# Circuitscape/Circuitscape.jl

Measured on AMD Instinct MI355X. Metric: pair-solves/sec (AMG-PCG, setup amortised over 100 pairs) on 10000x10000 raster pairwise, higher is better.
Workload: dtype f64

## Files before the change

circuitscape.jl_amd/csrc/lattice.h:

```cpp
#pragma once
#include "stencil.h"

namespace csgpu {

__device__ __forceinline__ int lat_tile(int i, int nc) {
  const int t = i / 3;
  return t < nc ? t : nc - 1;
}

template <class T>
__global__ __launch_bounds__(256) void lattice_q_fill_kernel(int64_t n, int R, int Rc, int Cc, const int* __restrict__ agg,
                                                             const int* __restrict__ qrp, const int* __restrict__ qci,
                                                             const T* __restrict__ qva, T* __restrict__ q,
                                                             int* __restrict__ bad) {
  for (int64_t node = (int64_t)blockIdx.x * 256 + threadIdx.x; node < n; node += (int64_t)gridDim.x * 256) {
    const int i = (int)(node % R), j = (int)(node / R);
    const int I = lat_tile(i, Rc), J = lat_tile(j, Cc);
    {
      const int a = agg[node];
      const int dI = a % Rc - I, dJ = a / Rc - J;
      if (dI < -1 || dI > 1 || dJ < -1 || dJ > 1) {
        atomicOr(bad, 1);
        continue;
      }
    }
    T row[9];
#pragma unroll
    for (int s = 0; s < 9; ++s) row[s] = T(0);
    for (int k = qrp[node]; k < qrp[node + 1]; ++k) {
      const int c = qci[k];
      const int dI = c % Rc - I, dJ = c / Rc - J;
      if (dI < -1 || dI > 1 || dJ < -1 || dJ > 1) {
        atomicOr(bad, 2);
        continue;
      }
      const int slot = (dJ + 1) * 3 + (dI + 1);
#pragma unroll
      for (int s = 0; s < 9; ++s)
        if (s == slot) row[s] = qva[k];
    }
#pragma unroll
    for (int s = 0; s < 9; ++s) q[node * 9 + s] = row[s];
  }
}

template <class T>
inline bool lattice_q_from_csr(const Csr<T>& Q, const int* agg, int R, int C, LatticeQ<T>& out, hipStream_t st) {
  const int64_t n = (int64_t)R * C;
  const int Rc = (R + 1) / 3, Cc = (C + 1) / 3;
  if (Q.nrows != n || Rc < 2 || Cc < 2 || (int64_t)Rc * Cc != Q.ncols) return false;
  DBuf q((size_t)n * 9 * sizeof(T));
  DBuf bad = dalloc<int>(1);
  CS_HIP(hipMemsetAsync(bad.p, 0, sizeof(int), st));
  hipLaunchKernelGGL((lattice_q_fill_kernel<T>), dim3(grid_for(n)), dim3(256), 0, st, n, R, Rc, Cc, agg, Q.rp(), Q.ci(),
                     Q.va(), dptr<T>(q), dptr<int>(bad));
  check_launch("index-free Q");
  if (read_int(dptr<int>(bad), st) != 0) return false;
  out.n = n;
  out.R = R;
  out.C = C;
  out.Rc = Rc;
  out.Cc = Cc;
  out.q = std::move(q);
  return true;
}

template <class T>
struct RestrictArgs {
  int R, C, Rc, Cc;
  int nstrips, nseg, segc;
  const T* q;
  const T* b;
  T* bc;
  const int* skip;
};

template <class T, int K, int NT>
struct RestrictShape {
  static constexpr int VEC = 16 / (int)sizeof(T);
  static constexpr int CPL = K < VEC ? K : VEC;
  static constexpr int LPR = K / CPL;
  static constexpr int TIC = NT / LPR;
  static constexpr int FR = 3 * TIC + 8;
  static constexpr int BU = (FR * LPR + NT - 1) / NT;
  static constexpr int QU = (FR * 9 + NT - 1) / NT;
};

template <class T, int K, int NT>
__global__ __launch_bounds__(NT) void lattice_restrict_kernel(RestrictArgs<T> a) {
  typedef RestrictShape<T, K, NT> SH;
  constexpr int CPL = SH::CPL, LPR = SH::LPR, TIC = SH::TIC, FR = SH::FR, BU = SH::BU, QU = SH::QU;
  typedef SpmvVec<T, CPL> XV;
  __shared__ XV s_b[3][FR * LPR];
  __shared__ T s_q[3][FR * 9];
  if (a.skip && *a.skip) return;
  const int tid = threadIdx.x;
  const int t = tid / LPR, lq = tid % LPR, c0 = lq * CPL;
  const int ntiles = a.nstrips * a.nseg;
  int t_first = blockIdx.x, t_last = ntiles, t_step = gridDim.x;
  if ((gridDim.x & 7) == 0) {
    const int xcd = blockIdx.x & 7, chunk = (ntiles + 7) >> 3;
    t_first = xcd * chunk + (blockIdx.x >> 3);
    t_last = min(ntiles, (xcd + 1) * chunk);
    t_step = gridDim.x >> 3;
  }
  for (int tile = t_first; tile < t_last; tile += t_step) {
    const int si = tile % a.nstrips, sj = tile / a.nstrips;
    const int Ic0 = si * TIC;
    const int Jc0 = sj * a.segc, Jc1 = min(a.Cc, Jc0 + a.segc);
    const int Ic = Ic0 + t;
    const bool row_on = Ic < a.Rc;
    const int f0 = max(3 * (Ic0 - 1), 0);
    const int last_tile = min(Ic0 + TIC, a.Rc - 1);
    const int f1 = last_tile >= a.Rc - 1 ? a.R : 3 * last_tile + 3;
    const int nfr = f1 - f0;
    const int fc0 = max(3 * (Jc0 - 1), 0);
    const int fc1 = Jc1 >= a.Cc - 1 ? a.C : 3 * Jc1 + 3;
    int rlo[3], rhi[3];
#pragma unroll
    for (int d = 0; d < 3; ++d) {
      const int tI = Ic - 1 + d;
      const bool on = row_on && tI >= 0 && tI < a.Rc;
      rlo[d] = on ? 3 * tI - f0 : 0;
      rhi[d] = on ? (tI >= a.Rc - 1 ? a.R : 3 * tI + 3) - f0 : 0;
    }
    XV breg[BU];
    T qreg[QU];
    auto load_column = [&](int f) {
      const int64_t base = (int64_t)f * a.R + f0;
#pragma unroll
      for (int u = 0; u < BU; ++u) {
        const int e = tid + u * NT;
        XV v;
#pragma unroll
        for (int q = 0; q < CPL; ++q) v.e[q] = T(0);
        if (e < nfr * LPR) v = *reinterpret_cast<const XV*>(a.b + (size_t)(base + e / LPR) * K + (e % LPR) * CPL);
        breg[u] = v;
      }
#pragma unroll
      for (int u = 0; u < QU; ++u) {
        const int e = tid + u * NT;
        qreg[u] = e < nfr * 9 ? a.q[base * 9 + e] : T(0);
      }
    };
    auto store_column = [&](int f) {
      const int slot = f % 3;
#pragma unroll
      for (int u = 0; u < BU; ++u) {
        const int e = tid + u * NT;
        if (e < FR * LPR) s_b[slot][e] = breg[u];
      }
#pragma unroll
      for (int u = 0; u < QU; ++u) {
        const int e = tid + u * NT;
        if (e < FR * 9) s_q[slot][e] = qreg[u];
      }
    };
    T acc[3][CPL];
#pragma unroll
    for (int d = 0; d < 3; ++d)
#pragma unroll
      for (int q = 0; q < CPL; ++q) acc[d][q] = T(0);
    auto emit = [&](int Jc, const T* v) {
      if (row_on && Jc >= Jc0 && Jc < Jc1) {
        XV o;
#pragma unroll
        for (int q = 0; q < CPL; ++q) o.e[q] = v[q];
        *reinterpret_cast<XV*>(a.bc + ((size_t)Jc * a.Rc + Ic) * K + c0) = o;
      }
    };
    __syncthreads();
    load_column(fc0);
    int Jf = lat_tile(fc0, a.Cc);
    for (int f = fc0; f < fc1; ++f) {
      store_column(f);
      if (f + 1 < fc1) load_column(f + 1);
      __syncthreads();
      const int Jn = lat_tile(f, a.Cc);
      if (Jn != Jf) {
        emit(Jf - 1, acc[0]);
#pragma unroll
        for (int q = 0; q < CPL; ++q) {
          acc[0][q] = acc[1][q];
          acc[1][q] = acc[2][q];
          acc[2][q] = T(0);
        }
        Jf = Jn;
      }
      const XV* sb = s_b[f % 3];
      const T* sq = s_q[f % 3];
#pragma unroll
      for (int d = 0; d < 3; ++d) {
        const int sI = (1 - d) + 1;
        for (int r = rlo[d]; r < rhi[d]; ++r) {
          const XV bv = sb[r * LPR + lq];
          const T* qr = sq + r * 9;
          const T wm = qr[0 * 3 + sI];
          const T w0 = qr[1 * 3 + sI];
          const T wp = qr[2 * 3 + sI];
#pragma unroll
          for (int q = 0; q < CPL; ++q) {
            acc[0][q] = fma(wm, bv.e[q], acc[0][q]);
            acc[1][q] = fma(w0, bv.e[q], acc[1][q]);
            acc[2][q] = fma(wp, bv.e[q], acc[2][q]);
          }
        }
      }
    }
    emit(Jf - 1, acc[0]);
    emit(Jf, acc[1]);
    emit(Jf + 1, acc[2]);
  }
}

inline int lattice_segc() {
  const int v = knobs().restrict_seg;
  return v < 2 ? 2 : v;
}

template <class T>
struct RupdRestrictOpts {
  const int* restart = nullptr;
  const int* src = nullptr;
  const int* dst = nullptr;
  const int* isrc = nullptr;
  const int* idst = nullptr;
  int icols = 0;
  T* xsol = nullptr;
};

template <class T>
struct RupdRestrictArgs : RupdRestrictOpts<T> {
  int64_t n;
  int R, C, Rc, Cc;
  int nstrips, nseg, segc;
  const T* rows;
  const T* q;
  const T* p;
  const T* r_in = nullptr;
  T* r_out;
  T* bc;
  const CgScalars* S = nullptr;
  double* partials = nullptr;
  const int* skip = nullptr;
};

template <class T, int K, int NT>
struct RupdRestrictShape {
  typedef RestrictShape<T, K, NT> RS;
  static constexpr int CPL = RS::CPL, LPR = RS::LPR, TIC = RS::TIC, FR = RS::FR;
  static constexpr int PR = FR + 2;
  static constexpr int RG = NT / LPR;
  static constexpr int BU = (FR + RG - 1) / RG;
  static constexpr int PU = (PR * LPR + NT - 1) / NT;
  static constexpr int MU = (PR * 5 + NT - 1) / NT;
  static constexpr int QU = (FR * 9 + NT - 1) / NT;
  static constexpr size_t lds_bytes = (size_t)3 * PR * LPR * 16 + (size_t)3 * PR * 5 * sizeof(T) + (size_t)FR * LPR * 16 +
                                      (size_t)FR * 9 * sizeof(T) + (size_t)(NT / 64) * K * sizeof(double);
};

template <class T, int K, int NT, bool APPLY = false, bool XUP = false>
__global__ __launch_bounds__(NT) void lattice_rupd_restrict_kernel(RupdRestrictArgs<T> a) {
  static_assert(!(APPLY && XUP), "the solution update belongs to the residual update");
  typedef RupdRestrictShape<T, K, NT> SH;
  constexpr int CPL = SH::CPL, LPR = SH::LPR, TIC = SH::TIC, FR = SH::FR, PR = SH::PR, BU = SH::BU, PU = SH::PU, MU = SH::MU,
                QU = SH::QU;
  typedef SpmvVec<T, CPL> XV;
  __shared__ XV s_p[3][PR * LPR];
  __shared__ T s_m[3][PR * 5];
  __shared__ XV s_b[FR * LPR];
  __shared__ T s_q[FR * 9];
  __shared__ double s_red[APPLY ? 1 : (NT / 64) * K];
  if (a.S && a.S->all_done) return;
  if (a.skip && *a.skip) return;
  const int tid = threadIdx.x;
  const int t = tid / LPR, lq = tid % LPR, c0 = lq * CPL;
  const int row0 = t * BU;
  T alpha[CPL];
#pragma unroll
  for (int qq = 0; qq < CPL; ++qq) alpha[qq] = APPLY ? T(0) : (T)a.S->alpha[c0 + qq];
  double dot_acc[CPL];
  bool fresh[CPL];
  int64_t nsrc[CPL], ndst[CPL];
#pragma unroll
  for (int qq = 0; qq < CPL; ++qq) {
    dot_acc[qq] = 0.0;
    fresh[qq] = !APPLY && !XUP && a.restart && a.restart[c0 + qq] != 0;
    nsrc[qq] = fresh[qq] ? a.src[c0 + qq] : -1;
    ndst[qq] = fresh[qq] ? a.dst[c0 + qq] : -1;
    if (nsrc[qq] == ndst[qq]) nsrc[qq] = ndst[qq] = -1;
  }
  const bool synth_in = !APPLY && !XUP && a.isrc != nullptr;
  int64_t is_[CPL], id_[CPL];
#pragma unroll
  for (int qq = 0; qq < CPL; ++qq) {
    const bool on = synth_in && c0 + qq < a.icols && a.isrc[c0 + qq] != a.idst[c0 + qq];
    is_[qq] = on ? a.isrc[c0 + qq] : -1;
    id_[qq] = on ? a.idst[c0 + qq] : -1;
  }
  const int ntiles = a.nstrips * a.nseg;
  int t_first = blockIdx.x, t_last = ntiles, t_step = gridDim.x;
  if ((gridDim.x & 7) == 0) {
    const int xcd = blockIdx.x & 7, chunk = (ntiles + 7) >> 3;
    t_first = xcd * chunk + (blockIdx.x >> 3);
    t_last = min(ntiles, (xcd + 1) * chunk);
    t_step = gridDim.x >> 3;
  }
  for (int tile = t_first; tile < t_last; tile += t_step) {
    const int si = tile % a.nstrips, sj = tile / a.nstrips;
    const int Ic0 = si * TIC;
    const int Jc0 = sj * a.segc, Jc1 = min(a.Cc, Jc0 + a.segc);
    const int Ic = Ic0 + t;
    const bool row_on = Ic < a.Rc;
    const int f0 = max(3 * (Ic0 - 1), 0);
    const int last_tile = min(Ic0 + TIC, a.Rc - 1);
    const int f1 = last_tile >= a.Rc - 1 ? a.R : 3 * last_tile + 3;
    const int nfr = f1 - f0;
    const int fc0 = max(3 * (Jc0 - 1), 0);
    const int fc1 = Jc1 >= a.Cc - 1 ? a.C : 3 * Jc1 + 3;
    const int o0 = 3 * Ic0, o1 = (Ic0 + TIC >= a.Rc) ? a.R : 3 * (Ic0 + TIC);
    const int oc0 = 3 * Jc0, oc1 = (Jc1 >= a.Cc) ? a.C : 3 * Jc1;
    int rlo[3], rhi[3];
#pragma unroll
    for (int d = 0; d < 3; ++d) {
      const int tI = Ic - 1 + d;
      const bool on = row_on && tI >= 0 && tI < a.Rc;
      rlo[d] = on ? 3 * tI - f0 : 0;
      rhi[d] = on ? (tI >= a.Rc - 1 ? a.R : 3 * tI + 3) - f0 : 0;
    }
    XV preg[PU];
    T mreg[MU];
    XV rreg[BU];
    XV xreg[XUP ? BU : 1];
    T qreg[QU];
    auto load_pm = [&](int f) {
      const int64_t base = (int64_t)f * a.R + f0 - 1;
#pragma unroll
      for (int u = 0; u < PU; ++u) {
        const int e = tid + u * NT;
        XV v;
#pragma unroll
        for (int qq = 0; qq < CPL; ++qq) v.e[qq] = T(0);
        const int64_t id = base + e / LPR;
        if (e < (nfr + 2) * LPR && id >= 0 && id < a.n) v = *reinterpret_cast<const XV*>(a.p + (size_t)id * K + (e % LPR) * CPL);
        preg[u] = v;
      }
#pragma unroll
      for (int u = 0; u < MU; ++u) {
        const int e = tid + u * NT;
        const int64_t g = base * 5 + e;
        mreg[u] = (e < (nfr + 2) * 5 && g >= 0 && g < a.n * 5) ? a.rows[g] : T(0);
      }
    };
    auto store_pm = [&](int slot) {
#pragma unroll
      for (int u = 0; u < PU; ++u) {
        const int e = tid + u * NT;
        if (e < PR * LPR) s_p[slot][e] = preg[u];
      }
#pragma unroll
      for (int u = 0; u < MU; ++u) {
        const int e = tid + u * NT;
        if (e < PR * 5) s_m[slot][e] = mreg[u];
      }
    };
    auto load_rq = [&](int f) {
      const int64_t base = (int64_t)f * a.R + f0;
#pragma unroll
      for (int u = 0; u < BU; ++u) {
        const int row = row0 + u;
        XV v;
#pragma unroll
        for (int qq = 0; qq < CPL; ++qq) v.e[qq] = T(0);
        if (!APPLY && f < fc1 && row < nfr) {
          const int64_t id = base + row;
          if (synth_in) {
#pragma unroll
            for (int qq = 0; qq < CPL; ++qq) v.e[qq] = id == is_[qq] ? T(-1) : (id == id_[qq] ? T(1) : T(0));
          } else {
            v = *reinterpret_cast<const XV*>(a.r_in + (size_t)id * K + c0);
          }
        }
        rreg[u] = v;
        if constexpr (XUP) {
          XV xv;
#pragma unroll
          for (int qq = 0; qq < CPL; ++qq) xv.e[qq] = T(0);
          const int fr = f0 + row;
          if (f >= oc0 && f < oc1 && row < nfr && fr >= o0 && fr < o1)
            xv = *reinterpret_cast<const XV*>(a.xsol + (size_t)(base + row) * K + c0);
          xreg[u] = xv;
        }
      }
#pragma unroll
      for (int u = 0; u < QU; ++u) {
        const int e = tid + u * NT;
        qreg[u] = (f < fc1 && e < nfr * 9) ? a.q[base * 9 + e] : T(0);
      }
    };
    T acc[3][CPL];
#pragma unroll
    for (int d = 0; d < 3; ++d)
#pragma unroll
      for (int qq = 0; qq < CPL; ++qq) acc[d][qq] = T(0);
    auto emit = [&](int Jc, const T* v) {
      if (row_on && Jc >= Jc0 && Jc < Jc1) {
        XV o;
#pragma unroll
        for (int qq = 0; qq < CPL; ++qq) o.e[qq] = v[qq];
        *reinterpret_cast<XV*>(a.bc + ((size_t)Jc * a.Rc + Ic) * K + c0) = o;
      }
    };
    __syncthreads();
    load_pm(fc0 - 1);
    store_pm(0);
    load_pm(fc0);
    store_pm(1);
    load_pm(fc0 + 1);
    load_rq(fc0);
    int Jf = lat_tile(fc0, a.Cc);
    int sm = 0, sc = 1, sp = 2;
    for (int f = fc0; f < fc1; ++f) {
      store_pm(sp);
      load_pm(f + 2);
      XV rv[BU];
      XV xv[XUP ? BU : 1];
      T qv[QU];
#pragma unroll
      for (int u = 0; u < BU; ++u) rv[u] = rreg[u];
      if constexpr (XUP) {
#pragma unroll
        for (int u = 0; u < BU; ++u) xv[u] = xreg[u];
      }
#pragma unroll
      for (int u = 0; u < QU; ++u) qv[u] = qreg[u];
      load_rq(f + 1);
      __syncthreads();
      const T* mp = s_m[sm];
      const T* mc = s_m[sc];
      const XV* xm = s_p[sm];
      const XV* x0 = s_p[sc];
      const XV* xp = s_p[sp];
      const bool col_owned = f >= oc0 && f < oc1;
      T sacc[BU][CPL];
      XV ctr[BU];
#pragma unroll
      for (int dj = 0; dj < 3; ++dj) {
        const XV* xcol = dj == 0 ? xm : (dj == 1 ? x0 : xp);
        XV win[BU + 2];
#pragma unroll
        for (int k = 0; k < BU + 2; ++k) {
#pragma unroll
          for (int qq = 0; qq < CPL; ++qq) win[k].e[qq] = T(0);
          if (row0 + k < nfr + 2) win[k] = xcol[(row0 + k) * LPR + lq];
        }
#pragma unroll
        for (int u = 0; u < BU; ++u) {
          const int row = row0 + u;
          if (row < nfr) {
            const int me = 5 * (row + 1);
            T w0, w1, w2;
            if (dj == 0) {
              w0 = mp[me - 5 + 4];
              w1 = mp[me + 3];
              w2 = mp[me + 5 + 2];
            } else if (dj == 1) {
              w0 = mc[me - 5 + 1];
              w1 = mc[me + 0];
              w2 = mc[me + 1];
            } else {
              w0 = mc[me + 2];
              w1 = mc[me + 3];
              w2 = mc[me + 4];
            }
#pragma unroll
            for (int qq = 0; qq < CPL; ++qq) {
              T sv = dj == 0 ? w0 * win[u].e[qq] : fma(w0, win[u].e[qq], sacc[u][qq]);
              sv = fma(w1, win[u + 1].e[qq], sv);
              sacc[u][qq] = fma(w2, win[u + 2].e[qq], sv);
            }
            if (dj == 1) ctr[u] = win[u + 1];
          }
        }
      }
#pragma unroll
      for (int u = 0; u < BU; ++u) {
        const int row = row0 + u;
        if (row < nfr) {
          XV rn;
#pragma unroll
          for (int qq = 0; qq < CPL; ++qq)
            rn.e[qq] = APPLY ? sacc[u][qq] : (fresh[qq] ? T(0) : rv[u].e[qq] - alpha[qq] * sacc[u][qq]);
          const int fr = f0 + row;
          const bool owned = col_owned && fr >= o0 && fr < o1;
          if (owned) {
#pragma unroll
            for (int qq = 0; qq < CPL; ++qq) dot_acc[qq] += (double)rn.e[qq] * (double)rn.e[qq];
          }
          const int64_t id = (int64_t)f * a.R + fr;
#pragma unroll
          for (int qq = 0; qq < CPL; ++qq)
            if (fresh[qq]) rn.e[qq] = id == nsrc[qq] ? T(-1) : (id == ndst[qq] ? T(1) : T(0));
          s_b[row * LPR + lq] = APPLY ? ctr[u] : rn;
          if (owned) dia_store(reinterpret_cast<XV*>(a.r_out + (size_t)id * K + c0), rn);
          if constexpr (XUP) {
            if (owned) {
              XV xn;
              const XV pc = x0[(row + 1) * LPR + lq];
#pragma unroll
              for (int qq = 0; qq < CPL; ++qq) xn.e[qq] = fma(alpha[qq], pc.e[qq], xv[u].e[qq]);
              dia_store(reinterpret_cast<XV*>(a.xsol + (size_t)id * K + c0), xn);
            }
          }
        }
      }
#pragma unroll
      for (int u = 0; u < QU; ++u) {
        const int e = tid + u * NT;
        if (e < FR * 9) s_q[e] = qv[u];
      }
      __syncthreads();
      const int Jn = lat_tile(f, a.Cc);
      if (Jn != Jf) {
        emit(Jf - 1, acc[0]);
#pragma unroll
        for (int qq = 0; qq < CPL; ++qq) {
          acc[0][qq] = acc[1][qq];
          acc[1][qq] = acc[2][qq];
          acc[2][qq] = T(0);
        }
        Jf = Jn;
      }
#pragma unroll
      for (int d = 0; d < 3; ++d) {
        const int sI = (1 - d) + 1;
        for (int r = rlo[d]; r < rhi[d]; ++r) {
          const XV bv = s_b[r * LPR + lq];
          const T* qr = s_q + r * 9;
          const T wm = qr[0 * 3 + sI];
          const T w0 = qr[1 * 3 + sI];
          const T wp = qr[2 * 3 + sI];
#pragma unroll
          for (int qq = 0; qq < CPL; ++qq) {
            acc[0][qq] = fma(wm, bv.e[qq], acc[0][qq]);
            acc[1][qq] = fma(w0, bv.e[qq], acc[1][qq]);
            acc[2][qq] = fma(wp, bv.e[qq], acc[2][qq]);
          }
        }
      }
      const int s0 = sm;
      sm = sc;
      sc = sp;
      sp = s0;
    }
    emit(Jf - 1, acc[0]);
    emit(Jf, acc[1]);
    emit(Jf + 1, acc[2]);
  }
  if (APPLY || !a.partials) return;
  if constexpr (!APPLY) {
    const int lane = tid & 63, w = tid >> 6;
    __syncthreads();
#pragma unroll
    for (int qq = 0; qq < CPL; ++qq) {
      double v = dot_acc[qq];
#pragma unroll
      for (int o = 32; o >= LPR; o >>= 1) v += __shfl_xor(v, o, 64);
      if (lane < LPR) s_red[w * K + lane * CPL + qq] = v;
    }
    __syncthreads();
    if (tid < K) {
      double ssum = 0.0;
#pragma unroll
      for (int ww = 0; ww < NT / 64; ++ww) ssum += s_red[ww * K + tid];
      a.partials[(size_t)blockIdx.x * K + tid] = ssum;
    }
  }
}

#ifndef CSGPU_FUSED_NT
#define CSGPU_FUSED_NT 512
#endif
constexpr int kFusedNT = CSGPU_FUSED_NT;
template <class T, int K>
constexpr bool lattice_rupd_restrict_fits() {
  return K >= 16 && RupdRestrictShape<T, K, kFusedNT>::lds_bytes <= (kFusedNT >= 512 ? 160 : 80) * 1024;
}

template <class T, int K>
inline int lattice_rupd_restrict_grid(const LatticeQ<T>& Q, int& nstrips, int& nseg, int& segc) {
  constexpr int NT = kFusedNT;
  segc = std::min(std::max(knobs().fused_seg, 2), Q.Cc);
  nstrips = ceil_div(Q.Rc, RestrictShape<T, K, NT>::TIC);
  while (segc > 16 && (int64_t)nstrips * ceil_div(Q.Cc, segc) < 1024) segc /= 2;
  nseg = ceil_div(Q.Cc, segc);
  int64_t g = (int64_t)nstrips * nseg;
  if (g > 16384) g = 16384;
  if (g >= 64) g &= ~(int64_t)7;
  return (int)std::max<int64_t>(g, 1);
}

template <class T, int K>
inline int lattice_rupd_args(const Dia<T>& D, const LatticeQ<T>& Q, const T* p, T* r_out, T* bc, RupdRestrictArgs<T>& a) {
  a.n = D.n;
  a.R = Q.R;
  a.C = Q.C;
  a.Rc = Q.Rc;
  a.Cc = Q.Cc;
  a.rows = D.data();
  a.q = Q.data();
  a.p = p;
  a.r_out = r_out;
  a.bc = bc;
  return lattice_rupd_restrict_grid<T, K>(Q, a.nstrips, a.nseg, a.segc);
}

template <class T, int K>
inline int lattice_rupd_restrict(const Dia<T>& D, const LatticeQ<T>& Q, const CgScalars* S, const T* p, const T* r_in, T* r_out,
                                 T* bc, double* partials, hipStream_t st, const RupdRestrictOpts<T>& o = RupdRestrictOpts<T>()) {
  CS_REQUIRE(!o.xsol || (!o.restart && !o.src && !o.dst && !o.isrc && !o.idst), CSGPU_INTERNAL,
             "fused residual update: the solution update takes a stored residual");
  if constexpr (!lattice_rupd_restrict_fits<T, K>()) {
    return 0;
  } else {
    RupdRestrictArgs<T> a;
    const int g = lattice_rupd_args<T, K>(D, Q, p, r_out, bc, a);
    a.r_in = r_in;
    a.S = S;
    a.partials = partials;
    static_cast<RupdRestrictOpts<T>&>(a) = o;
    if (o.xsol)
      hipLaunchKernelGGL((lattice_rupd_restrict_kernel<T, K, kFusedNT, false, true>), dim3(g), dim3(kFusedNT), 0, st, a);
    else
      hipLaunchKernelGGL((lattice_rupd_restrict_kernel<T, K, kFusedNT>), dim3(g), dim3(kFusedNT), 0, st, a);
    return partials ? g : 0;
  }
}

template <class T, int K>
inline bool lattice_apply_restrict(const Dia<T>& D, const LatticeQ<T>& Q, const T* x, T* y, T* bc, const int* skip,
                                   hipStream_t st) {
  if constexpr (!lattice_rupd_restrict_fits<T, K>()) {
    return false;
  } else {
    RupdRestrictArgs<T> a;
    const int g = lattice_rupd_args<T, K>(D, Q, x, y, bc, a);
    a.skip = skip;
    hipLaunchKernelGGL((lattice_rupd_restrict_kernel<T, K, kFusedNT, true>), dim3(g), dim3(kFusedNT), 0, st, a);
    return true;
  }
}

template <class T, int K>
__global__ __launch_bounds__(64) void lattice_restrict_pairs_kernel(int R, int Rc, int Cc, const T* __restrict__ q,
                                                                    const int* __restrict__ src, const int* __restrict__ dst,
                                                                    int ncols, T* __restrict__ bc) {
  const int c = threadIdx.x;
  if (c >= ncols || c >= K || src[c] == dst[c]) return;
#pragma unroll 1
  for (int which = 0; which < 2; ++which) {
    const int64_t node = which == 0 ? src[c] : dst[c];
    const T sign = which == 0 ? T(-1) : T(1);
    const int i = (int)(node % R), j = (int)(node / R);
    const int I = lat_tile(i, Rc), J = lat_tile(j, Cc);
    for (int dj = 0; dj < 3; ++dj)
      for (int di = 0; di < 3; ++di) {
        const int Ic = I + di - 1, Jc = J + dj - 1;
        if (Ic < 0 || Ic >= Rc || Jc < 0 || Jc >= Cc) continue;
        const T w = q[(size_t)node * 9 + dj * 3 + di];
        T* at = bc + ((size_t)Jc * Rc + Ic) * K + c;
        *at = fma(w, sign, *at);
      }
  }
}

template <class T, int K>
inline void lattice_restrict_pairs(const LatticeQ<T>& Q, const int* src, const int* dst, int ncols, T* bc, hipStream_t st) {
  CS_HIP(hipMemsetAsync(bc, 0, (size_t)Q.Rc * Q.Cc * K * sizeof(T), st));
  hipLaunchKernelGGL((lattice_restrict_pairs_kernel<T, K>), dim3(1), dim3(64), 0, st, Q.R, Q.Rc, Q.Cc, Q.data(), src, dst, ncols,
                     bc);
}

template <class T, int K>
inline void lattice_restrict(const LatticeQ<T>& Q, const T* b, T* bc, const int* skip, hipStream_t st) {
  constexpr int NT = 128;
  RestrictArgs<T> a;
  a.R = Q.R;
  a.C = Q.C;
  a.Rc = Q.Rc;
  a.Cc = Q.Cc;
  a.segc = std::min(lattice_segc(), Q.Cc);
  a.nstrips = ceil_div(Q.Rc, RestrictShape<T, K, NT>::TIC);
  a.nseg = ceil_div(Q.Cc, a.segc);
  a.q = Q.data();
  a.b = b;
  a.bc = bc;
  a.skip = skip;
  int64_t g = (int64_t)a.nstrips * a.nseg;
  if (g > 65536) g = 65536;
  if (g >= 64) g &= ~(int64_t)7;
  hipLaunchKernelGGL((lattice_restrict_kernel<T, K, NT>), dim3((int)std::max<int64_t>(g, 1)), dim3(NT), 0, st, a);
}

}
```

circuitscape.jl_amd/csrc/stencil.h:

```cpp
#pragma once
#include "blas1.h"
#include "spmv.h"

namespace csgpu {

#ifndef CSGPU_DIA_NT
#define CSGPU_DIA_NT 0
#endif
template <class T, int N>
__device__ __forceinline__ void dia_store(SpmvVec<T, N>* p, const SpmvVec<T, N>& v) {
#if CSGPU_DIA_NT >= 1 && defined(__HIPCC__)
  typedef T VT __attribute__((ext_vector_type(N)));
  VT t;
#pragma unroll
  for (int q = 0; q < N; ++q) t[q] = v.e[q];
  __builtin_nontemporal_store(t, reinterpret_cast<VT*>(p));
#else
  *p = v;
#endif
}
template <class T, int N>
__device__ __forceinline__ SpmvVec<T, N> dia_load(const SpmvVec<T, N>* p) {
#if CSGPU_DIA_NT >= 2 && defined(__HIPCC__)
  typedef T VT __attribute__((ext_vector_type(N)));
  const VT t = __builtin_nontemporal_load(reinterpret_cast<const VT*>(p));
  SpmvVec<T, N> v;
#pragma unroll
  for (int q = 0; q < N; ++q) v.e[q] = t[q];
  return v;
#else
  return *p;
#endif
}


__device__ __forceinline__ int dia_slot(int64_t d, int R) {
  if (d == 0) return 0;
  if (d == 1) return 1;
  if (d == R - 1) return 2;
  if (d == R) return 3;
  if (d == R + 1) return 4;
  return -1;
}

template <class T>
__global__ __launch_bounds__(256) void dia_fill_kernel(int n, int R, const int* __restrict__ rp,
                                                       const int* __restrict__ ci, const T* __restrict__ va,
                                                       T* __restrict__ rows, int* __restrict__ bad) {
  for (int i = blockIdx.x * 256 + threadIdx.x; i < n; i += gridDim.x * 256) {
    for (int k = rp[i]; k < rp[i + 1]; ++k) {
      const int64_t d = (int64_t)ci[k] - i;
      const int s = dia_slot(d < 0 ? -d : d, R);
      if (s < 0) {
        atomicOr(bad, 1);
        continue;
      }
      if (d >= 0) rows[(size_t)i * 5 + s] = va[k];
    }
  }
}

template <class T>
__global__ __launch_bounds__(256) void dia_check_kernel(int n, int R, const int* __restrict__ rp,
                                                        const int* __restrict__ ci, const T* __restrict__ va,
                                                        const T* __restrict__ rows, int* __restrict__ bad) {
  for (int i = blockIdx.x * 256 + threadIdx.x; i < n; i += gridDim.x * 256) {
    for (int k = rp[i]; k < rp[i + 1]; ++k) {
      const int64_t d = (int64_t)ci[k] - i;
      if (d >= 0) continue;
      const int s = dia_slot(-d, R);
      if (s < 0 || !(rows[(size_t)ci[k] * 5 + s] == va[k])) atomicOr(bad, 1);
    }
  }
}

template <class T>
inline bool dia_from_csr(const Csr<T>& A, int R, Dia<T>& out, hipStream_t st, bool trusted = false) {
  const int n = A.nrows;
  if (A.nrows != A.ncols || R < 4 || n < 4 * R || (n % R) != 0) return false;
  DBuf rows((size_t)n * 5 * sizeof(T));
  DBuf bad = dalloc<int>(1);
  CS_HIP(hipMemsetAsync(rows.p, 0, rows.bytes, st));
  CS_HIP(hipMemsetAsync(bad.p, 0, sizeof(int), st));
  const int g = grid_for(n);
  hipLaunchKernelGGL((dia_fill_kernel<T>), dim3(g), dim3(256), 0, st, n, R, A.rp(), A.ci(), A.va(), dptr<T>(rows),
                     dptr<int>(bad));
  if (!trusted)
    hipLaunchKernelGGL((dia_check_kernel<T>), dim3(g), dim3(256), 0, st, n, R, A.rp(), A.ci(), A.va(),
                       (const T*)dptr<T>(rows), dptr<int>(bad));
  check_launch("lattice form");
  if (read_int(dptr<int>(bad), st) != 0) return false;
  out.n = n;
  out.R = R;
  out.rows = std::move(rows);
  return true;
}

enum DiaMode {
  DIA_PLAIN = 0,
  DIA_CG = 1,
  DIA_SQP = 4,
  DIA_SQ = 2,
  DIA_RUPD = 3
};

template <class T, class XT>
struct DiaArgs {
  int64_t n;
  int R, C;
  int nstrips, nseg, seg;
  const T* rows;
  const CgScalars* S;
  const XT* z;
  const XT* pin;
  XT* pout;
  T* y;
  double* partials;
  const double* beta_dev;
  const int* skip;
  const T* qell;
  int Rc, Cc;
  const XT* xc;
  T* r;
  XT* rp;
  T* xsol;
  const int* restart = nullptr;
  const T* bsub = nullptr;
  const T* xadd = nullptr;
  const int* psrc = nullptr;
  const int* pdst = nullptr;
  int pcols = 0;
};

template <class T, class XT, int K>
struct DiaShape {
  static constexpr int VEC = 16 / (int)sizeof(XT);
  static constexpr int CPL = K < VEC ? K : VEC;
  static constexpr int LPR = K / CPL;
  static constexpr int TI = 256 / LPR;
  static constexpr int MELEMS = 5 * (TI + 2);
  static constexpr int MU = (MELEMS + 255) / 256;
  static constexpr int QELEMS = 9 * TI;
  static constexpr int QU = (QELEMS + 255) / 256;
  static constexpr int CR = TI / 3 + 4;
};

#ifndef CSGPU_RUPD_WAVES
#define CSGPU_RUPD_WAVES 1
#endif
template <class T, class XT, int K, int MODE>
__global__ __launch_bounds__(256, ((MODE == DIA_CG && K >= 8) ? 4 : ((MODE == DIA_RUPD && K >= 32) ? CSGPU_RUPD_WAVES : 1))) void dia_cg_kernel(
    DiaArgs<T, XT> a) {
  constexpr bool FUSE = MODE == DIA_CG;
  typedef DiaShape<T, XT, K> SH;
  constexpr int CPL = SH::CPL, LPR = SH::LPR, TI = SH::TI, MELEMS = SH::MELEMS, MU = SH::MU;
  typedef SpmvVec<XT, CPL> XV;
  typedef SpmvVec<T, CPL> YV;
  constexpr int QELEMS = SH::QELEMS, QU = SH::QU, CR = SH::CR;
  constexpr bool SQ = MODE == DIA_SQ || MODE == DIA_SQP;
  constexpr bool SYNTH = MODE == DIA_SQP;
  static_assert(CR * LPR <= 256, "one lane per staged coarse entry");
  __shared__ XV s_x[4][(TI + 2) * LPR];
  __shared__ T s_m[4][MELEMS];
  __shared__ T s_q[SQ ? 4 : 1][SQ ? QELEMS : 1];
  __shared__ XV s_xc[SQ ? 4 : 1][SQ ? CR * LPR : 1];
  __shared__ double s_red[4 * K];
  if (a.S && a.S->all_done) return;
  if (a.skip && *a.skip) return;
  const int tid = threadIdx.x;
  const int t = tid / LPR;
  const int lq = tid % LPR;
  const int c0 = lq * CPL;
  T beta[CPL];
#pragma unroll
  for (int q = 0; q < CPL; ++q)
    beta[q] = FUSE ? (a.S ? (T)a.S->beta[c0 + q] : (a.beta_dev ? (T)a.beta_dev[c0 + q] : T(0))) : T(0);
  T alpha[CPL];
#pragma unroll
  for (int q = 0; q < CPL; ++q) alpha[q] = (MODE == DIA_RUPD) ? (T)a.S->alpha[c0 + q] : T(0);
  bool fresh[CPL];
#pragma unroll
  for (int q = 0; q < CPL; ++q) fresh[q] = (MODE == DIA_RUPD) && a.restart && a.restart[c0 + q] != 0;
  double dot_acc[CPL];
#pragma unroll
  for (int q = 0; q < CPL; ++q) dot_acc[q] = 0.0;
  int64_t ps[SYNTH ? CPL : 1], pd[SYNTH ? CPL : 1];
  if (SYNTH) {
#pragma unroll
    for (int q = 0; q < CPL; ++q) {
      const bool on = c0 + q < a.pcols && a.psrc[c0 + q] != a.pdst[c0 + q];
      ps[q] = on ? a.psrc[c0 + q] : -1;
      pd[q] = on ? a.pdst[c0 + q] : -1;
    }
  }
  auto synth = [&](int64_t id) {
    XV v;
#pragma unroll
    for (int q = 0; q < CPL; ++q) v.e[q] = id == ps[SYNTH ? q : 0] ? XT(-1) : (id == pd[SYNTH ? q : 0] ? XT(1) : XT(0));
    return v;
  };

  const int ntiles = a.nstrips * a.nseg;
  int t_first = blockIdx.x, t_last = ntiles, t_step = gridDim.x;
  if ((gridDim.x & 7) == 0) {
    const int xcd = blockIdx.x & 7, chunk = (ntiles + 7) >> 3;
    t_first = xcd * chunk + (blockIdx.x >> 3);
    t_last = min(ntiles, (xcd + 1) * chunk);
    t_step = gridDim.x >> 3;
  }
  for (int tile = t_first; tile < t_last; tile += t_step) {
    const int si = tile % a.nstrips, sj = tile / a.nstrips;
    const int i0 = si * TI;
    const int j0 = sj * a.seg, j1 = min(a.C, j0 + a.seg);
    const bool row_on = i0 + t < a.R;
    const int Ilo = SQ ? min(i0 / 3, a.Rc - 1) - 1 : 0;
    const int crow = SQ ? min((i0 + t) / 3, a.Rc - 1) - Ilo : 0;
    XV xr, xh;
    XV zr, zh;
    T mr[MU];
    T qr[SQ ? QU : 1];
    XV xcr;
    const bool have_pin = !FUSE || a.pin != nullptr;
    YV r_pre;
    int pend_c = -1, next_c = 0;
    auto load_r = [&](int jc) {
#pragma unroll
      for (int q = 0; q < CPL; ++q) r_pre.e[q] = T(0);
      const int64_t id = (int64_t)jc * a.R + i0 + t;
      if (MODE == DIA_RUPD && jc < j1 && row_on && id < a.n) r_pre = dia_load(reinterpret_cast<const YV*>(a.r + (size_t)id * K + c0));
    };
    auto load_coarse = [&](int Jc) {
#pragma unroll
      for (int q = 0; q < CPL; ++q) xcr.e[q] = XT(0);
      if (tid < CR * LPR) {
        const int Ic = Ilo + tid / LPR;
        if (Jc >= 0 && Jc < a.Cc && Ic >= 0 && Ic < a.Rc)
          xcr = *reinterpret_cast<const XV*>(a.xc + ((size_t)Jc * a.Rc + Ic) * K + (tid % LPR) * CPL);
      }
    };
    auto store_coarse = [&](int Jc) {
      if (tid < CR * LPR) s_xc[Jc & 3][tid] = xcr;
    };
    auto load_column = [&](int jc) {
      const int64_t base = (int64_t)jc * a.R + i0 - 1;
      {
        const int64_t id = base + 1 + t;
#pragma unroll
        for (int q = 0; q < CPL; ++q) {
          xr.e[q] = XT(0);
          zr.e[q] = XT(0);
        }
        if (id >= 0 && id < a.n) {
          const size_t e = (size_t)id * K + c0;
          if (SYNTH) xr = synth(id);
          else if (have_pin) xr = *reinterpret_cast<const XV*>(a.pin + e);
          if (FUSE) zr = dia_load(reinterpret_cast<const XV*>(a.z + e));
        }
      }
      if (tid < 2 * LPR) {
        const int64_t id = base + (tid < LPR ? 0 : TI + 1);
#pragma unroll
        for (int q = 0; q < CPL; ++q) {
          xh.e[q] = XT(0);
          zh.e[q] = XT(0);
        }
        if (id >= 0 && id < a.n) {
          const size_t e = (size_t)id * K + c0;
          if (SYNTH) xh = synth(id);
          else if (have_pin) xh = *reinterpret_cast<const XV*>(a.pin + e);
          if (FUSE) zh = *reinterpret_cast<const XV*>(a.z + e);
        }
      }
#pragma unroll
      for (int u = 0; u < MU; ++u) {
        const int e = tid + u * 256;
        const int64_t g = base * 5 + e;
        mr[u] = (e < MELEMS && g >= 0 && g < a.n * 5) ? a.rows[g] : T(0);
      }
      if (SQ) {
        const int64_t qb = ((int64_t)(jc - 1) * a.R + i0) * 9;
#pragma unroll
        for (int u = 0; u < QU; ++u) {
          const int e = tid + u * 256;
          const int64_t g = qb + e;
          qr[u] = (jc - 1 >= j0 && e < QELEMS && g < a.n * 9) ? a.qell[g] : T(0);
        }
      }
    };
    auto store_column = [&](int jc) {
      const int slot = jc & 3;
      if (FUSE) {
        XV v;
#pragma unroll
        for (int q = 0; q < CPL; ++q) v.e[q] = (beta[q] == T(0) || !have_pin) ? zr.e[q] : (XT)fma(beta[q], (T)xr.e[q], (T)zr.e[q]);
        const int64_t id = (int64_t)jc * a.R + i0 + t;
        if (jc >= j0 && jc < j1 && row_on && id < a.n) dia_store(reinterpret_cast<XV*>(a.pout + (size_t)id * K + c0), v);
        xr = v;
#pragma unroll
        for (int q = 0; q < CPL; ++q) xh.e[q] = (beta[q] == T(0) || !have_pin) ? zh.e[q] : (XT)fma(beta[q], (T)xh.e[q], (T)zh.e[q]);
      }
      s_x[slot][(t + 1) * LPR + lq] = xr;
      if (tid < 2 * LPR) s_x[slot][(tid < LPR ? 0 : TI + 1) * LPR + lq] = xh;
#pragma unroll
      for (int u = 0; u < MU; ++u) {
        const int e = tid + u * 256;
        if (e < MELEMS) s_m[slot][e] = mr[u];
      }
      if (SQ) {
#pragma unroll
        for (int u = 0; u < QU; ++u) {
          const int e = tid + u * 256;
          if (e < QELEMS) s_q[(jc - 1) & 3][e] = qr[u];
        }
      }
    };
    __syncthreads();
    load_column(j0 - 1);
    store_column(j0 - 1);
    load_column(j0);
    store_column(j0);
    load_column(j0 + 1);
    if (MODE == DIA_RUPD) load_r(j0);
    if (SQ) {
      const int Jb = min(j0 / 3, a.Cc - 1);
      for (int d = -1; d <= 2; ++d) {
        load_coarse(Jb + d);
        store_coarse(Jb + d);
      }
      next_c = Jb + 3;
    }
    __syncthreads();
    XV xw[3][3];
#pragma unroll
    for (int di = 0; di < 3; ++di) {
      xw[1][di] = s_x[(j0 - 1) & 3][(t + di) * LPR + lq];
      xw[2][di] = s_x[j0 & 3][(t + di) * LPR + lq];
    }
// ... 603 lines not shown
```

Measured before the change: 53.72.

## Use AMDGPU buffer loads/stores with hardware bounds checks in fused residual-restrict kernel

Replaces the per-element bounds-checked global loads and stores in the lattice residual-update/restrict kernel with raw buffer resource loads and stores. The hardware range check returns zero out of bounds and drops out-of-range writes, which removes the explicit branch conditions. Per-column source and destination ids move from registers into shared memory to cut register pressure. The kernel also fixes the accumulation trip counts for interior strips and tracks the coarse-column advance incrementally instead of dividing. This relies on 32-bit offsets and buffer descriptor semantics and adds scheduling fences, so correctness now depends on the offset arithmetic staying within bounds.

```diff
diff --git a/circuitscape.jl_amd/csrc/lattice.h b/circuitscape.jl_amd/csrc/lattice.h
--- a/circuitscape.jl_amd/csrc/lattice.h
+++ b/circuitscape.jl_amd/csrc/lattice.h
@@ -276,27 +276,34 @@
   const int tid = threadIdx.x;
   const int t = tid / LPR, lq = tid % LPR, c0 = lq * CPL;
   const int row0 = t * BU;
+  static_assert(FR % BU == 0, "a thread's adjacent rows are all staged or none is");
+  static_assert(LPR * 16 == K * (int)sizeof(T), "a K-wide row is LPR 16-byte vectors");
+  constexpr uint32_t ROWB = LPR * 16;
+  const bool active = row0 < FR;
+  const uint32_t voff_row = (uint32_t)row0 * ROWB + lq * 16;
   T alpha[CPL];
 #pragma unroll
   for (int qq = 0; qq < CPL; ++qq) alpha[qq] = APPLY ? T(0) : (T)a.S->alpha[c0 + qq];
   double dot_acc[CPL];
   bool fresh[CPL];
-  int64_t nsrc[CPL], ndst[CPL];
+  __shared__ int64_t s_ids[(APPLY || XUP) ? 1 : 4][(APPLY || XUP) ? 1 : K];
+  const bool synth_in = !APPLY && !XUP && a.isrc != nullptr;
 #pragma unroll
   for (int qq = 0; qq < CPL; ++qq) {
     dot_acc[qq] = 0.0;
     fresh[qq] = !APPLY && !XUP && a.restart && a.restart[c0 + qq] != 0;
-    nsrc[qq] = fresh[qq] ? a.src[c0 + qq] : -1;
-    ndst[qq] = fresh[qq] ? a.dst[c0 + qq] : -1;
-    if (nsrc[qq] == ndst[qq]) nsrc[qq] = ndst[qq] = -1;
-  }
-  const bool synth_in = !APPLY && !XUP && a.isrc != nullptr;
-  int64_t is_[CPL], id_[CPL];
-#pragma unroll
-  for (int qq = 0; qq < CPL; ++qq) {
-    const bool on = synth_in && c0 + qq < a.icols && a.isrc[c0 + qq] != a.idst[c0 + qq];
-    is_[qq] = on ? a.isrc[c0 + qq] : -1;
-    id_[qq] = on ? a.idst[c0 + qq] : -1;
+    if constexpr (!APPLY && !XUP) {
+      int64_t nsrc = fresh[qq] ? a.src[c0 + qq] : -1;
+      int64_t ndst = fresh[qq] ? a.dst[c0 + qq] : -1;
+      if (nsrc == ndst) nsrc = ndst = -1;
+      const bool on = synth_in && c0 + qq < a.icols && a.isrc[c0 + qq] != a.idst[c0 + qq];
+      if (t == 0) {
+        s_ids[0][c0 + qq] = nsrc;
+        s_ids[1][c0 + qq] = ndst;
+        s_ids[2][c0 + qq] = on ? a.isrc[c0 + qq] : -1;
+        s_ids[3][c0 + qq] = on ? a.idst[c0 + qq] : -1;
+      }
+    }
   }
   const int ntiles = a.nstrips * a.nseg;
   int t_first = blockIdx.x, t_last = ntiles, t_step = gridDim.x;
@@ -330,27 +337,27 @@
     }
     XV preg[PU];
     T mreg[MU];
-    XV rreg[BU];
+    XV rreg[BU] = {};
     XV xreg[XUP ? BU : 1];
     T qreg[QU];
-    auto load_pm = [&](int f) {
-      const int64_t base = (int64_t)f * a.R + f0 - 1;
-#pragma unroll
-      for (int u = 0; u < PU; ++u) {
-        const int e = tid + u * NT;
-        XV v;
-#pragma unroll
-        for (int qq = 0; qq < CPL; ++qq) v.e[qq] = T(0);
-        const int64_t id = base + e / LPR;
-        if (e < (nfr + 2) * LPR && id >= 0 && id < a.n) v = *reinterpret_cast<const XV*>(a.p + (size_t)id * K + (e % LPR) * CPL);
-        preg[u] = v;
-      }
-#pragma unroll
-      for (int u = 0; u < MU; ++u) {
-        const int e = tid + u * NT;
-        const int64_t g = base * 5 + e;
-        mreg[u] = (e < (nfr + 2) * 5 && g >= 0 && g < a.n * 5) ? a.rows[g] : T(0);
-      }
+    const uint32_t own_shift = (uint32_t)(o0 - f0) * ROWB, own_rows = (uint32_t)(o1 - o0);
+    auto load_pm = [&](int f, auto lead_form) {
+      constexpr bool LEAD = decltype(lead_form)::value;
+      int64_t base = (int64_t)f * a.R + f0 - 1;
+      const int64_t end = std::min<int64_t>(base + nfr + 2, a.n);
+      uint32_t lead = 0;
+      if (LEAD && base < 0) {
+        lead = (uint32_t)std::min<int64_t>(-base, nfr + 2);
+        base += lead;
+      }
+      const uint32_t etid = opaque((uint32_t)tid);
+      const BufRun bp = buf_run(a.p + base * K, (end - base) * (int64_t)ROWB);
+      const BufRun bm = buf_run(a.rows + base * 5, (end - base) * (int64_t)(5 * sizeof(T)));
+#pragma unroll
+      for (int u = 0; u < PU; ++u) preg[u] = buf_load<XV>(bp, (etid + u * NT) * 16u - lead * ROWB);
+#pragma unroll
+      for (int u = 0; u < MU; ++u)
+        mreg[u] = buf_load<T>(bm, (etid + u * NT) * (uint32_t)sizeof(T) - lead * (uint32_t)(5 * sizeof(T)));
     };
     auto store_pm = [&](int slot) {
 #pragma unroll
@@ -366,37 +373,29 @@
     };
     auto load_rq = [&](int f) {
       const int64_t base = (int64_t)f * a.R + f0;
-#pragma unroll
-      for (int u = 0; u < BU; ++u) {
-        const int row = row0 + u;
-        XV v;
-#pragma unroll
-        for (int qq = 0; qq < CPL; ++qq) v.e[qq] = T(0);
-        if (!APPLY && f < fc1 && row < nfr) {
-          const int64_t id = base + row;
-          if (synth_in) {
-#pragma unroll
-            for (int qq = 0; qq < CPL; ++qq) v.e[qq] = id == is_[qq] ? T(-1) : (id == id_[qq] ? T(1) : T(0));
-          } else {
-            v = *reinterpret_cast<const XV*>(a.r_in + (size_t)id * K + c0);
-          }
-        }
-        rreg[u] = v;
-        if constexpr (XUP) {
-          XV xv;
-#pragma unroll
-          for (int qq = 0; qq < CPL; ++qq) xv.e[qq] = T(0);
-          const int fr = f0 + row;
-          if (f >= oc0 && f < oc1 && row < nfr && fr >= o0 && fr < o1)
-            xv = *reinterpret_cast<const XV*>(a.xsol + (size_t)(base + row) * K + c0);
-          xreg[u] = xv;
-        }
-      }
-#pragma unroll
-      for (int u = 0; u < QU; ++u) {
-        const int e = tid + u * NT;
-        qreg[u] = (f < fc1 && e < nfr * 9) ? a.q[base * 9 + e] : T(0);
-      }
+      const int rows = f < fc1 ? nfr : 0;
+      const uint32_t etid = opaque((uint32_t)tid), vrow = opaque(voff_row), vown = vrow - own_shift;
+      if (!APPLY && synth_in) {
+#pragma unroll
+        for (int u = 0; u < BU; ++u) {
+          const int64_t id = base + row0 + u;
+#pragma unroll
+          for (int qq = 0; qq < CPL; ++qq)
+            rreg[u].e[qq] = row0 + u < rows ? (id == s_ids[2][c0 + qq] ? T(-1) : (id == s_ids[3][c0 + qq] ? T(1) : T(0))) : T(0);
+        }
+      } else if (!APPLY) {
+        const BufRun br = buf_run(a.r_in + base * K, (int64_t)rows * ROWB);
+#pragma unroll
+        for (int u = 0; u < BU; ++u) rreg[u] = buf_load<XV>(br, vrow + u * ROWB);
+      }
+      if constexpr (XUP) {
+        const BufRun bx = buf_run(a.xsol + ((int64_t)f * a.R + o0) * K, f >= oc0 && f < oc1 ? (int64_t)(o1 - o0) * ROWB : 0);
+#pragma unroll
+        for (int u = 0; u < BU; ++u) xreg[u] = buf_load<XV>(bx, vown + u * ROWB);
+      }
+      const BufRun bq = buf_run(a.q + base * 9, (int64_t)rows * (int64_t)(9 * sizeof(T)));
+#pragma unroll
+      for (int u = 0; u < QU; ++u) qreg[u] = buf_load<T>(bq, (etid + u * NT) * (uint32_t)sizeof(T));
     };
     T acc[3][CPL];
 #pragma unroll
@@ -412,17 +411,19 @@
       }
     };
     __syncthreads();
-    load_pm(fc0 - 1);
+    load_pm(fc0 - 1, std::true_type());
     store_pm(0);
-    load_pm(fc0);
+    load_pm(fc0, std::true_type());
     store_pm(1);
-    load_pm(fc0 + 1);
+    load_pm(fc0 + 1, std::false_type());
     load_rq(fc0);
     int Jf = lat_tile(fc0, a.Cc);
+    int fnext = 3 * (Jf + 1);
     int sm = 0, sc = 1, sp = 2;
+    const bool regular = sizeof(T) == 8 && Ic0 + TIC < a.Rc - 1;
     for (int f = fc0; f < fc1; ++f) {
       store_pm(sp);
-      load_pm(f + 2);
+      load_pm(f + 2, std::false_type());
       XV rv[BU];
       XV xv[XUP ? BU : 1];
       T qv[QU];
@@ -442,23 +443,19 @@
       const XV* x0 = s_p[sc];
       const XV* xp = s_p[sp];
       const bool col_owned = f >= oc0 && f < oc1;
-      T sacc[BU][CPL];
-      XV ctr[BU];
-#pragma unroll
-      for (int dj = 0; dj < 3; ++dj) {
-        const XV* xcol = dj == 0 ? xm : (dj == 1 ? x0 : xp);
-        XV win[BU + 2];
-#pragma unroll
-        for (int k = 0; k < BU + 2; ++k) {
-#pragma unroll
-          for (int qq = 0; qq < CPL; ++qq) win[k].e[qq] = T(0);
-          if (row0 + k < nfr + 2) win[k] = xcol[(row0 + k) * LPR + lq];
-        }
-#pragma unroll
-        for (int u = 0; u < BU; ++u) {
-          const int row = row0 + u;
-          if (row < nfr) {
-            const int me = 5 * (row + 1);
+      if (active) {
+        T sacc[BU][CPL];
+        XV ctr[BU];
+#pragma unroll
+        for (int dj = 0; dj < 3; ++dj) {
+          sched_fence();
+          const XV* xcol = dj == 0 ? xm : (dj == 1 ? x0 : xp);
+          XV win[BU + 2];
+#pragma unroll
+          for (int k = 0; k < BU + 2; ++k) win[k] = xcol[(row0 + k) * LPR + lq];
+#pragma unroll
+          for (int u = 0; u < BU; ++u) {
+            const int me = 5 * (row0 + u + 1);
             T w0, w1, w2;
             if (dj == 0) {
               w0 = mp[me - 5 + 4];
@@ -482,35 +479,44 @@
             if (dj == 1) ctr[u] = win[u + 1];
           }
         }
-      }
-#pragma unroll
-      for (int u = 0; u < BU; ++u) {
-        const int row = row0 + u;
-        if (row < nfr) {
+        const int64_t own_id = (int64_t)f * a.R + o0;
+        const int64_t own_bytes = col_owned ? (int64_t)(o1 - o0) * ROWB : 0;
+        const uint32_t vown = opaque(voff_row) - own_shift;
+        const BufRun bo = buf_run(a.r_out + own_id * K, own_bytes);
+        const BufRun bx = buf_run(XUP ? a.xsol + own_id * K : nullptr, XUP ? own_bytes : 0);
+        int64_t nsrc[CPL], ndst[CPL];
+#pragma unroll
+        for (int qq = 0; qq < CPL; ++qq) {
+          nsrc[qq] = (APPLY || XUP) ? -1 : s_ids[0][(APPLY || XUP) ? 0 : c0 + qq];
+          ndst[qq] = (APPLY || XUP) ? -1 : s_ids[1][(APPLY || XUP) ? 0 : c0 + qq];
+        }
+#pragma unroll
+        for (int u = 0; u < BU; ++u) {
+          const int row = row0 + u;
           XV rn;
 #pragma unroll
           for (int qq = 0; qq < CPL; ++qq)
             rn.e[qq] = APPLY ? sacc[u][qq] : (fresh[qq] ? T(0) : rv[u].e[qq] - alpha[qq] * sacc[u][qq]);
-          const int fr = f0 + row;
-          const bool owned = col_owned && fr >= o0 && fr < o1;
-          if (owned) {
-#pragma unroll
-            for (int qq = 0; qq < CPL; ++qq) dot_acc[qq] += (double)rn.e[qq] * (double)rn.e[qq];
+          if constexpr (!APPLY) {
+            if (col_owned && (uint32_t)(row - (o0 - f0)) < own_rows) {
+#pragma unroll
+              for (int qq = 0; qq < CPL; ++qq) dot_acc[qq] += (double)rn.e[qq] * (double)rn.e[qq];
+            }
+            {
+              const int64_t id = (int64_t)f * a.R + f0 + row;
+#pragma unroll
+              for (int qq = 0; qq < CPL; ++qq)
+                if (fresh[qq]) rn.e[qq] = id == nsrc[qq] ? T(-1) : (id == ndst[qq] ? T(1) : T(0));
+            }
           }
-          const int64_t id = (int64_t)f * a.R + fr;
-#pragma unroll
-          for (int qq = 0; qq < CPL; ++qq)
-            if (fresh[qq]) rn.e[qq] = id == nsrc[qq] ? T(-1) : (id == ndst[qq] ? T(1) : T(0));
           s_b[row * LPR + lq] = APPLY ? ctr[u] : rn;
-          if (owned) dia_store(reinterpret_cast<XV*>(a.r_out + (size_t)id * K + c0), rn);
+          buf_store(bo, vown + u * ROWB, rn);
           if constexpr (XUP) {
-            if (owned) {
-              XV xn;
-              const XV pc = x0[(row + 1) * LPR + lq];
-#pragma unroll
-              for (int qq = 0; qq < CPL; ++qq) xn.e[qq] = fma(alpha[qq], pc.e[qq], xv[u].e[qq]);
-              dia_store(reinterpret_cast<XV*>(a.xsol + (size_t)id * K + c0), xn);
-            }
+            XV xn;
+            const XV pc = x0[(row + 1) * LPR + lq];
+#pragma unroll
+            for (int qq = 0; qq < CPL; ++qq) xn.e[qq] = fma(alpha[qq], pc.e[qq], xv[u].e[qq]);
+            buf_store(bx, vown + u * ROWB, xn);
           }
         }
       }
@@ -520,8 +526,7 @@
         if (e < FR * 9) s_q[e] = qv[u];
       }
       __syncthreads();
-      const int Jn = lat_tile(f, a.Cc);
-      if (Jn != Jf) {
+      if (f == fnext && Jf + 1 < a.Cc) {
         emit(Jf - 1, acc[0]);
 #pragma unroll
         for (int qq = 0; qq < CPL; ++qq) {
@@ -529,24 +534,34 @@
           acc[1][qq] = acc[2][qq];
           acc[2][qq] = T(0);
         }
-        Jf = Jn;
-      }
-#pragma unroll
-      for (int d = 0; d < 3; ++d) {
-        const int sI = (1 - d) + 1;
-        for (int r = rlo[d]; r < rhi[d]; ++r) {
-          const XV bv = s_b[r * LPR + lq];
-          const T* qr = s_q + r * 9;
-          const T wm = qr[0 * 3 + sI];
-          const T w0 = qr[1 * 3 + sI];
-          const T wp = qr[2 * 3 + sI];
-#pragma unroll
-          for (int qq = 0; qq < CPL; ++qq) {
-            acc[0][qq] = fma(wm, bv.e[qq], acc[0][qq]);
-            acc[1][qq] = fma(w0, bv.e[qq], acc[1][qq]);
-            acc[2][qq] = fma(wp, bv.e[qq], acc[2][qq]);
+        ++Jf;
+        fnext += 3;
+      }
+      auto acc_row = [&](int r, int sI) {
+        const XV bv = s_b[r * LPR + lq];
+        const T* qr = s_q + r * 9;
+        const T wm = qr[0 * 3 + sI];
+        const T w0 = qr[1 * 3 + sI];
+        const T wp = qr[2 * 3 + sI];
+#pragma unroll
+        for (int qq = 0; qq < CPL; ++qq) {
+          acc[0][qq] = fma(wm, bv.e[qq], acc[0][qq]);
+          acc[1][qq] = fma(w0, bv.e[qq], acc[1][qq]);
+          acc[2][qq] = fma(wp, bv.e[qq], acc[2][qq]);
+        }
+      };
+      if (regular) {
+#pragma unroll
+        for (int d = 0; d < 3; ++d) {
+          if (d > 0 || rhi[0] > rlo[0]) {
+#pragma unroll
+            for (int k = 0; k < 3; ++k) acc_row(rlo[1] + 3 * (d - 1) + k, (1 - d) + 1);
           }
         }
+      } else {
+#pragma unroll
+        for (int d = 0; d < 3; ++d)
+          for (int r = rlo[d]; r < rhi[d]; ++r) acc_row(r, (1 - d) + 1);
       }
       const int s0 = sm;
       sm = sc;
diff --git a/circuitscape.jl_amd/csrc/stencil.h b/circuitscape.jl_amd/csrc/stencil.h
--- a/circuitscape.jl_amd/csrc/stencil.h
+++ b/circuitscape.jl_amd/csrc/stencil.h
@@ -33,6 +33,73 @@
 #endif
 }
 
+struct BufRun {
+#if defined(__HIPCC__)
+  __amdgpu_buffer_rsrc_t rs;
+#else
+  const char* base;
+  uint32_t bytes;
+#endif
+};
+__device__ __forceinline__ BufRun buf_run(const void* base, int64_t bytes) {
+  BufRun b;
+  const int nb = bytes > 0 ? (int)bytes : 0;
+#if defined(__HIPCC__)
+  b.rs = __builtin_amdgcn_make_buffer_rsrc(const_cast<void*>(base), 0, nb, 0x00020000);
+#else
+  b.base = static_cast<const char*>(base);
+  b.bytes = (uint32_t)nb;
+#endif
+  return b;
+}
+template <class VT>
+__device__ __forceinline__ VT buf_load(const BufRun& b, uint32_t off) {
+  static_assert(sizeof(VT) == 16 || sizeof(VT) == 8 || sizeof(VT) == 4, "buffer loads are 4, 8 or 16 bytes wide");
+  VT v;
+#if defined(__HIPCC__)
+  if constexpr (sizeof(VT) == 16) {
+    const auto t = __builtin_amdgcn_raw_buffer_load_b128(b.rs, off, 0, 0);
+    __builtin_memcpy(&v, &t, 16);
+  } else if constexpr (sizeof(VT) == 8) {
+    const auto t = __builtin_amdgcn_raw_buffer_load_b64(b.rs, off, 0, 0);
+    __builtin_memcpy(&v, &t, 8);
+  } else {
+    const auto t = __builtin_amdgcn_raw_buffer_load_b32(b.rs, off, 0, 0);
+    __builtin_memcpy(&v, &t, 4);
+  }
+#else
+  if ((uint64_t)off + sizeof(VT) <= b.bytes)
+    memcpy(&v, b.base + off, sizeof(VT));
+  else
+    memset(&v, 0, sizeof(VT));
+#endif
+  return v;
+}
+template <class VT>
+__device__ __forceinline__ void buf_store(const BufRun& b, uint32_t off, const VT& v) {
+  static_assert(sizeof(VT) == 16, "buffer stores are 16 bytes wide");
+#if defined(__HIPCC__)
+  typedef unsigned int U4 __attribute__((ext_vector_type(4)));
+  U4 t;
+  __builtin_memcpy(&t, &v, 16);
+  __builtin_amdgcn_raw_buffer_store_b128(t, b.rs, off, 0, 0);
+#else
+  if ((uint64_t)off + sizeof(VT) <= b.bytes) memcpy(const_cast<char*>(b.base) + off, &v, sizeof(VT));
+#endif
+}
+
+__device__ __forceinline__ uint32_t opaque(uint32_t x) {
+#if defined(__HIPCC__) && defined(__HIP_DEVICE_COMPILE__)
+  asm volatile("" : "+v"(x));
+#endif
+  return x;
+}
+
+__device__ __forceinline__ void sched_fence() {
+#if defined(__HIPCC__) && defined(__HIP_DEVICE_COMPILE__)
+  __builtin_amdgcn_sched_barrier(0);
+#endif
+}
 
 __device__ __forceinline__ int dia_slot(int64_t d, int R) {
   if (d == 0) return 0;
```

After: 43.46. 0.809x the previous value.
